# eora-ai/torchok

Measured on AMD Instinct MI355X. Metric: images/sec (node) ResNet-50 224px bs256/GPU; step p50 ms, higher is better.
Workload: dtype bf16

## Files before the change

include/tok.h:

```cpp
#ifndef TOK_H_
#define TOK_H_

#include <stddef.h>
#include <stdint.h>

#ifdef __cplusplus
extern "C" {
#endif

typedef enum tok_status {
  TOK_OK = 0,
  TOK_ERR_INVALID = -1,
  TOK_ERR_LAUNCH = -2,
  TOK_ERR_WORKSPACE = -3
} tok_status;

typedef enum tok_dtype { TOK_F32 = 0, TOK_F16 = 1, TOK_BF16 = 2 } tok_dtype;

typedef struct tok_conv_desc {
  int32_t n, h, w, c;
  int32_t k;
  int32_t r, s;
  int32_t p, q;
  int32_t stride, pad;
// ... 23 lines not shown
  int32_t k, r, s, c, k_pad, s_pad, c_pad;
  int32_t block_start;
} tok_pack_item;
int tok_pack_item_blocks(const tok_pack_item* item );
int tok_pack_weights_batched(const tok_pack_item* items_dev, int n_items, int total_blocks, void* stream);


int tok_conv_fwd_stat_rows(const tok_conv_desc* d);
int tok_conv_fwd(const tok_conv_desc* d, const void* x, const void* w, const float* bias,
                 void* y, float* stats, void* stream);
int tok_conv_dgrad(const tok_conv_desc* d, const void* dy, const void* w_dgrad, void* dx,
                   int accumulate, void* stream);
int tok_conv_dgrad_stat_rows(const tok_conv_desc* d);
int tok_conv_dgrad_bnstats(const tok_conv_desc* d, const void* dy, const void* w_dgrad, void* dx,
                           int accumulate, const void* bn_y, const uint8_t* bn_mask, float* partial,
                           void* stream);
int tok_bn_gram_finalize(const float* Z, const float* zsum, const float* w, int64_t count, int p, int k,
                         const float* gamma, const float* beta, float* running_mean, float* running_var,
                         int64_t* num_batches_tracked, float momentum, float eps, float* mean, float* rstd,
                         float* scale, float* shift, float* wz ,
                         void* stream);
int tok_conv_fwd_bn_apply(const tok_conv_desc* d, const void* x, const void* w, const float* scale, const float* shift,
                          const void* shortcut , int relu, void* out, uint8_t* mask ,
                          void* stream);
int tok_conv_dgrad_maskstore(const tok_conv_desc* d, const void* dy, const void* w_dgrad, void* dx, int accumulate,
                             const uint8_t* mask, float* partial, void* stream);
int tok_relu_mask_reduce(const void* dout, const uint8_t* mask, int64_t m, int c, void* dz, float* partial, void* stream);
int tok_bn3_bwd_prepare(const float* G, const float* w, const float* wz, const float* zsum, const float* partial, int rows,
                        int64_t count, int p, int k, const float* gamma, const float* mean, const float* rstd,
                        float* dgamma, float* dbeta, int param_accumulate, float* coef, float* dw, int dw_accumulate,
                        void* wa, void* wb, float* cvec, float* ws ,
                        void* stream);
size_t tok_bn3_bwd_prepare_ws_floats(int p, int k);
int tok_conv_dgrad_bias(const tok_conv_desc* d, const void* dy, const void* w_dgrad, const float* bias, void* dx,
                        int accumulate, const void* bn_y, const uint8_t* bn_mask, float* partial, void* stream);
int tok_subsample2_fwd(const void* x, int n, int h, int w, int c, void* out, void* stream);
int tok_subsample2_bwd(const void* dsub, int n, int h, int w, int c, void* dx, int accumulate, void* stream);
int tok_conv_dgrad_subacc_ok(const tok_conv_desc* d);
int tok_conv_dgrad_subacc(const tok_conv_desc* d, const void* dy, const void* w_dgrad, void* dx, const void* dsub,
                          const void* bn_y , const uint8_t* mask ,
                          float* partial , int mask_store, void* stream);
int tok_conv_dgrad2_ok(const tok_conv_desc* d1, const tok_conv_desc* d2);
int tok_conv_dgrad2(const tok_conv_desc* d1, const void* dy1, const void* w1_dgrad, const tok_conv_desc* d2, const void* dy2,
                    const void* w2_dgrad, const float* bias , void* dx, int accumulate,
                    const void* bn_y , const uint8_t* bn_mask , float* partial ,
                    void* stream);
size_t tok_conv_wgrad_ws_bytes(const tok_conv_desc* d);
int tok_conv_wgrad(const tok_conv_desc* d, const void* x, const void* dy, float* dw,
                   int k_real, int c_real, void* ws, size_t ws_bytes, int accumulate,
                   void* stream);
int tok_conv_wgrad_bias_ok(const tok_conv_desc* d);
size_t tok_conv_wgrad_bias_ws_bytes(const tok_conv_desc* d);
int tok_conv_wgrad_bias(const tok_conv_desc* d, const void* x, const void* dy, float* dw, int k_real, int c_real,
                        void* ws, size_t ws_bytes, int accumulate, float* dbias, int bias_accumulate, void* stream);


int tok_bn_finalize(const float* stats, int rows, int64_t count, int c, int c_real,
                    const float* gamma, const float* beta,
                    float* running_mean, float* running_var, int64_t* nbt,
                    float momentum, float eps,
                    float* mean, float* rstd, float* scale, float* shift, void* stream);
int tok_bn_eval_coeffs(const float* gamma, const float* beta, const float* running_mean,
                       const float* running_var, float eps, int c, int c_real,
                       float* scale, float* shift, void* stream);
int tok_bn_stats_rows(int64_t m, int c);
int tok_bn_stats(const void* y, int64_t m, int c, float* stats, void* stream);
// ... 313 lines not shown
```

torchok_amd/_C.py:

```python
import ctypes
import os
from ctypes import POINTER, Structure, c_char_p, c_float, c_int, c_int32, c_int64, c_size_t, c_void_p

_HERE = os.path.dirname(os.path.abspath(__file__))
LIB_PATH = os.environ.get('TOK_LIB') or os.path.join(_HERE, 'lib', 'libtok_gfx950.so')

TOK_F32, TOK_F16, TOK_BF16 = 0, 1, 2
TOK_CE_LOSS_FLOATS = 2050


class ConvDesc(Structure):
    _fields_ = [('n', c_int32), ('h', c_int32), ('w', c_int32), ('c', c_int32),
                ('k', c_int32), ('r', c_int32), ('s', c_int32),
                ('p', c_int32), ('q', c_int32),
                ('stride', c_int32), ('pad', c_int32), ('s_pad', c_int32)]


class PackItem(Structure):
    _fields_ = [('src', c_void_p), ('dst_fwd', c_void_p), ('dst_dgrad', c_void_p),
                ('k', c_int32), ('r', c_int32), ('s', c_int32), ('c', c_int32),
                ('k_pad', c_int32), ('s_pad', c_int32), ('c_pad', c_int32), ('block_start', c_int32)]


TOK_GRAD_CLIP_MAX_PARTIALS = 1024
# ... 27 lines not shown
    'tok_bn_eval_coeffs': (c_int, [_P, _P, _P, _P, c_float, c_int, c_int, _P, _P, _P]),
    'tok_bn_stats_rows': (c_int, [c_int64, c_int]),
    'tok_bn_stats': (c_int, [_P, c_int64, c_int, _P, _P]),
    'tok_bn_act_fwd': (c_int, [_P, _P, _P, _P, c_int, _P, _P, c_int64, c_int, _P]),
    'tok_bn_act_fwd_colsum_rows': (c_int, [c_int64, c_int]),
    'tok_event_create': (_P, []),
    'tok_event_destroy': (c_int, [_P]),
    'tok_next_launch_event': (c_int, [_P]),
    'tok_stream_wait_event': (c_int, [_P, _P]),
    'tok_bn_act_fwd_colsum': (c_int, [_P, _P, _P, _P, c_int, _P, _P, c_int64, c_int, _P, _P]),
    'tok_bn_bwd_rows': (c_int, [c_int64, c_int]),
    'tok_bn_bwd_reduce': (c_int, [_P, _P, _P, _P, _P, _P, _P, c_int, c_int64, c_int, _P, _P]),
    'tok_bn_bwd_finalize': (c_int, [_P, c_int, c_int64, c_int, c_int, _P, _P, _P, _P, _P, _P, c_int, c_int, _P]),
    'tok_bn_bwd_apply': (c_int, [_P, _P, _P, _P, _P, _P, c_int, _P, _P, c_int, c_int64, c_int, _P]),
    'tok_bn_hswish_fwd': (c_int, [_P, _P, _P, _P, c_int64, c_int, _P]),
    'tok_bn_hswish_bwd_reduce': (c_int, [_P, _P, _P, _P, _P, _P, c_int64, c_int, _P, _P]),
    'tok_bn_hswish_bwd_apply': (c_int, [_P, _P, _P, _P, _P, _P, c_int64, c_int, _P]),
    'tok_maxpool3x3s2_fwd': (c_int, [_P, _P, _P, c_int, c_int, c_int, c_int, _P]),
    'tok_maxpool3x3s2_bwd': (c_int, [_P, _P, _P, c_int, c_int, c_int, c_int, c_int, _P]),
    'tok_avgpool2x2_fwd': (c_int, [_P, _P, c_int, c_int, c_int, c_int, _P]),
    'tok_avgpool2x2_bwd': (c_int, [_P, _P, c_int, c_int, c_int, c_int, c_int, _P]),
    'tok_gap_fwd': (c_int, [_P, _P, c_int, c_int, c_int, _P]),
    'tok_gap_bwd': (c_int, [_P, _P, c_int, c_int, c_int, c_int, _P]),
    'tok_global_pool_fwd': (c_int, [_P, _P, _P, c_int, c_int, c_int, c_int, c_int, _P]),
    'tok_global_pool_bwd': (c_int, [_P, _P, _P, c_int, c_int, c_int, c_int, c_int, c_int, _P]),
    'tok_colsum': (c_int, [_P, c_int64, c_int, c_int, _P, c_int, _P]),
    'tok_bn_gram_finalize': (c_int, [_P, _P, _P, c_int64, c_int, c_int, _P, _P, _P, _P, _P, c_float, c_float, _P, _P, _P, _P, _P, _P]),
    'tok_conv_fwd_bn_apply': (c_int, [POINTER(ConvDesc), _P, _P, _P, _P, _P, c_int, _P, _P, _P]),
    'tok_conv_dgrad_maskstore': (c_int, [POINTER(ConvDesc), _P, _P, _P, c_int, _P, _P, _P]),
    'tok_relu_mask_reduce': (c_int, [_P, _P, c_int64, c_int, _P, _P, _P]),
    'tok_bn3_bwd_prepare': (c_int, [_P, _P, _P, _P, _P, c_int, c_int64, c_int, c_int, _P, _P, _P, _P, _P, c_int, _P, _P, c_int,
                                    _P, _P, _P, _P, _P]),
    'tok_bn3_bwd_prepare_ws_floats': (c_size_t, [c_int, c_int]),
    'tok_conv_dgrad_bias': (c_int, [POINTER(ConvDesc), _P, _P, _P, _P, c_int, _P, _P, _P, _P]),
    'tok_conv_dgrad2_ok': (c_int, [POINTER(ConvDesc), POINTER(ConvDesc)]),
    'tok_conv_dgrad2': (c_int, [POINTER(ConvDesc), _P, _P, POINTER(ConvDesc), _P, _P, _P, _P, c_int, _P, _P, _P, _P]),
    'tok_subsample2_fwd': (c_int, [_P, c_int, c_int, c_int, c_int, _P, _P]),
    'tok_subsample2_bwd': (c_int, [_P, c_int, c_int, c_int, c_int, _P, c_int, _P]),
    'tok_conv_dgrad_subacc_ok': (c_int, [POINTER(ConvDesc)]),
    'tok_conv_dgrad_subacc': (c_int, [POINTER(ConvDesc), _P, _P, _P, _P, _P, _P, _P, c_int, _P]),
    'tok_softmax_ce_fwd': (c_int, [_P, _P, c_int, c_int, c_int, c_int64, _P, _P, _P, _P]),
    'tok_softmax_ce_bwd': (c_int, [_P, _P, _P, _P, _P, c_int, c_int, c_int, c_int64, _P, _P]),
    'tok_softmax_ce_smooth_fwd': (c_int, [_P, _P, c_int, c_int, c_int, c_int64, c_float, _P, _P, _P, _P]),
    'tok_softmax_ce_smooth_bwd': (c_int, [_P, _P, _P, _P, _P, c_int, c_int, c_int, c_int64, c_float, _P, _P]),
    'tok_upsample_ce_serves': (c_int, [c_int, c_int]),
    'tok_upsample_ce_fwd': (c_int, [_P, c_int, c_int, c_int, c_int, c_int, c_int, c_int, _P, c_int64, _P, _P, _P, _P]),
    'tok_upsample_ce_bwd': (c_int, [_P, c_int, c_int, c_int, c_int, c_int, c_int, c_int, _P, c_int64, _P, _P, _P, _P, c_int, _P]),
    'tok_dice_rows': (c_int, [c_int64]),
    'tok_dice_fwd': (c_int, [_P, _P, c_int64, c_int, c_int, c_int, c_float, c_float, c_int, _P, c_int, _P, _P, _P, _P]),
    'tok_dice_bwd': (c_int, [_P, _P, _P, _P, c_int64, c_int, c_int, c_int, _P, _P]),
    'tok_bce_logits_fwd': (c_int, [_P, _P, c_int64, c_int, c_int, c_float, c_int, _P, _P]),
    'tok_bce_logits_bwd': (c_int, [_P, _P, _P, _P, c_int64, c_int, c_int, c_float, c_int, _P, _P]),
    'tok_relevance_matrix_multilabel': (c_int, [_P, _P, c_int, c_int, c_int, _P, _P]),
    'tok_embed_reg_fwd': (c_int, [_P, c_int, c_int, c_int, c_int, _P, _P, _P]),
    'tok_embed_reg_bwd': (c_int, [_P, _P, _P, c_float, c_int, c_int, c_int, c_int, _P, _P]),
    'tok_regression_loss_fwd': (c_int, [_P, _P, c_int64, c_int, c_float, c_int, _P, _P]),
    'tok_regression_loss_bwd': (c_int, [_P, _P, _P, c_int64, c_int, c_float, c_int, _P, _P]),
    'tok_confusion_update': (c_int, [_P, _P, _P, c_int64, c_int, c_int, c_int64, _P, _P]),
    'tok_cls_stats_update': (c_int, [_P, _P, _P, c_int64, c_int, c_int, c_int64, _P, _P]),
    'tok_l2norm_fwd': (c_int, [_P, _P, _P, c_int, c_int, c_int, c_int, c_float, _P]),
    'tok_l2norm_bwd': (c_int, [_P, _P, _P, _P, c_int, c_int, c_int, c_int, c_int, _P]),
    'tok_arcface_margin_fwd': (c_int, [_P, _P, c_int, c_int, c_int, c_float, c_float, c_float, c_float, c_int, c_float, _P, _P]),
    'tok_arcface_margin_bwd': (c_int, [_P, _P, _P, c_int, c_int, c_int, c_float, c_float, c_float, c_float, c_int, c_float, _P, _P]),
    'tok_relevance_matrix': (c_int, [_P, _P, c_int, c_int, _P, _P]),
    'tok_contrastive_fwd': (c_int, [_P, _P, _P, c_int, c_int, c_int, c_int, c_float, _P, _P, _P, _P]),
    'tok_contrastive_bwd': (c_int, [_P, _P, _P, _P, _P, c_int, c_int, c_int, c_int, c_float, _P, _P, c_int, _P]),
# ... 136 lines not shown
```

torchok_amd/csrc/conv_common.h:

```cpp
#pragma once
#include "tok_common.h"

struct FastDiv {
  uint32_t mul, shift;
};
static inline FastDiv make_fastdiv(uint32_t d) {
  FastDiv f;
  if (d <= 1) { f.mul = 0; f.shift = 0; return f; }
  uint32_t l = 0;
  while ((1ull << l) < d) ++l;
  f.mul = (uint32_t)((((1ull << 32) * ((1ull << l) - d)) / d) + 1);
  f.shift = l;
  return f;
}
__device__ __forceinline__ uint32_t fdiv(uint32_t n, FastDiv f) {
  return (uint32_t)(((uint64_t)__umulhi(n, f.mul) + n) >> f.shift);
}

struct ConvArgs {
  const bf16* x;
  const bf16* w;
  bf16* y;
  const float* bias;
  float* stats;
// ... 17 lines not shown
  int stride, pad;
  int M, PQ, Ktot, KT;
  int gridM, gridN;
  int accumulate, uniform_taps;
  uint32_t x_bytes, w_bytes;
  uint32_t s_bytes;
  FastDiv fd_pq, fd_q;
  unsigned long long* timing;
  int stat_rows;
  int cls_M[4], cls_nw[4], cls_hw[4];
  FastDiv cls_fd_hw[4], cls_fd_w[4];
};


bool conv_win_serves(const ConvArgs& a);
int conv_win_grid(int gridM, int gridN);
void conv_win_tiles(const ConvArgs& a, int* gridM, int* gridN);
int conv_win_launch(ConvArgs& a, hipStream_t st);
bool conv_s2d_serves(const ConvArgs& a, int stride, int pad);
int conv_s2d_grid(int gridM, int gridN);
void conv_s2d_tiles(const ConvArgs& a, int* gridM, int* gridN);
int conv_s2d_launch(ConvArgs& a, hipStream_t st);

bool gemm256_geometry(const ConvArgs& a);
bool gemm256_modes(const ConvArgs& a);
bool gemm256_serves(const ConvArgs& a);
int gemm256_rows(const ConvArgs& a);
int gemm256_launch(ConvArgs& a, hipStream_t st);

bool stem_win_serves(const ConvArgs& a);
int stem_win_launch(ConvArgs& a, int stat_rows, hipStream_t st);
bool stem_wgrad_serves(const tok_conv_desc* d);
int stem_wgrad_launch(const tok_conv_desc* d, const void* x, const void* dy, float* ws, int slabs, hipStream_t st);
```

torchok_amd/csrc/conv_wgrad.hip:

```cpp
#include "tok_common.h"
#include "conv_common.h"
#include <type_traits>
#include <stdlib.h>

namespace {

struct WgradArgs {
  const bf16* x;
  const bf16* dy;
  float* ws;
  int H, W, C, K, R, S, P, Q, stride, pad;
  int M, PQ, HW, Ktot;
  int tilesN, tilesK, splitM, mchunk;
  uint32_t x_bytes, dy_bytes;
  uint32_t pq_mul, pq_shift, q_mul, q_shift;
  float* cs;
  int cs_cols;
  int adv_q, adv_p;
  size_t cs_stride, ws_stride;
};

__device__ __forceinline__ uint32_t magic_div(uint32_t n, uint32_t mul, uint32_t shift) {
  return (uint32_t)(((uint64_t)__umulhi(n, mul) + n) >> shift);
}
// ... 1131 lines not shown
    return true;
  }();
  (void)attr_set;
  hipLaunchKernelGGL((conv_wgrad_ring_kernel<TN, TK>), dim3(a.tilesN * a.tilesK * a.splitM), dim3(256), smem, st, a);
}

template <int TN, int TK, bool C4, int MS, bool PWK>
void launch_wgrad_pw(const WgradArgs& a, hipStream_t st) {
  constexpr int smem = 2 * MS * ((TN + 16) * 2 + (TK + 16) * 2);
  static const bool attr_set = [&] {
    (void)hipFuncSetAttribute(reinterpret_cast<const void*>(&conv_wgrad_kernel<TN, TK, C4, MS, PWK>),
                              hipFuncAttributeMaxDynamicSharedMemorySize, smem);
    return true;
  }();
  (void)attr_set;
  hipLaunchKernelGGL((conv_wgrad_kernel<TN, TK, C4, MS, PWK>), dim3(a.tilesN * a.tilesK * a.splitM), dim3(256),
                     smem, st, a);
}

template <int TN, int TK, bool C4, int MS>
void launch_wgrad_ms(const WgradArgs& a, hipStream_t st) {
  if constexpr (!C4) {
    if (a.R == 1 && a.S == 1 && a.stride == 1 && a.pad == 0) { launch_wgrad_pw<TN, TK, C4, MS, true>(a, st); return; }
  }
  launch_wgrad_pw<TN, TK, C4, MS, false>(a, st);
}

template <int TN, int TK, bool C4>
void launch_wgrad(const WgradArgs& a, hipStream_t st, int ms) {
  if (ms == 64) launch_wgrad_ms<TN, TK, C4, 64>(a, st);
  else launch_wgrad_ms<TN, TK, C4, 32>(a, st);
}

}

extern "C" size_t tok_conv_wgrad_ws_bytes(const tok_conv_desc* d) {
  if (d == nullptr) return 0;
  const Plan p = make_plan(d);
  return (size_t)p.splitM * d->k * d->r * d->s_pad * d->c * sizeof(float);
}

extern "C" int tok_conv_wgrad_bias_ok(const tok_conv_desc* d) {
  if (d == nullptr || d->c == 4) return 0;
  return make_plan(d).ring ? 1 : 0;
}

extern "C" size_t tok_conv_wgrad_bias_ws_bytes(const tok_conv_desc* d) {
  if (d == nullptr) return 0;
  const Plan p = make_plan(d);
  return tok_conv_wgrad_ws_bytes(d) + (size_t)p.splitM * d->k * sizeof(float);
}

namespace {
int wgrad_impl(const tok_conv_desc* d, const void* x, const void* dy, float* dw, int k_real, int c_real, void* ws, size_t ws_bytes,
               int accumulate, float* dbias, int bias_accumulate, void* stream);
}

extern "C" int tok_conv_wgrad(const tok_conv_desc* d, const void* x, const void* dy, float* dw,
                              int k_real, int c_real, void* ws, size_t ws_bytes, int accumulate,
                              void* stream) {
  return wgrad_impl(d, x, dy, dw, k_real, c_real, ws, ws_bytes, accumulate, nullptr, 0, stream);
}

extern "C" int tok_conv_wgrad_bias(const tok_conv_desc* d, const void* x, const void* dy, float* dw, int k_real, int c_real,
                                   void* ws, size_t ws_bytes, int accumulate, float* dbias, int bias_accumulate, void* stream) {
  TOK_CHECK_ARG(dbias != nullptr, "tok_conv_wgrad_bias: dbias must not be null");
// ... 122 lines not shown
```

torchok_amd/csrc/unit3.hip:

```cpp
#include "tok_common.h"

namespace {

__device__ __forceinline__ float round_bf16(float v) { return bf2f(f2bf(v)); }

template <bool TRANS_A, bool ROUND_A, bool ROUND_B>
__global__ __launch_bounds__(256) void gemm_f32_kernel(const float* __restrict__ A, int lda, const float* __restrict__ B, int ldb,
                                                       int M, int N, int L, float* __restrict__ C, int ldc, int epi, int split,
                                                       bf16* __restrict__ Cb, int ldcb, float* __restrict__ cvec) {
  __shared__ float As[16][64 + 4];
  __shared__ float Bs[16][64 + 4];
  const int tid = threadIdx.x;
  const int i0 = blockIdx.y * 64, j0 = blockIdx.x * 64;
  const int ti = tid >> 4, tj = tid & 15;
  const int lchunk = ((L + (int)gridDim.z - 1) / (int)gridDim.z + 15) / 16 * 16;
  const int lbeg = blockIdx.z * lchunk;
  const int lend = min(L, lbeg + lchunk);
  if (gridDim.z > 1) C += (size_t)blockIdx.z * M * ldc;
  float acc[4][4];
#pragma unroll
  for (int r = 0; r < 4; ++r)
#pragma unroll
    for (int c = 0; c < 4; ++c) acc[r][c] = 0.f;
  for (int l0 = lbeg; l0 < lend; l0 += 16) {
#pragma unroll
    for (int e = 0; e < 4; ++e) {
      const int idx = tid + e * 256;
      int ii, ll;
      if (TRANS_A) { ii = idx & 63; ll = idx >> 6; }
      else { ll = idx & 15; ii = idx >> 4; }
      const int gi = i0 + ii, gl = l0 + ll;
      float v = 0.f;
      if (gi < M && gl < lend) v = TRANS_A ? A[(size_t)gl * lda + gi] : A[(size_t)gi * lda + gl];
// ... 278 lines not shown
    const float m1 = (float)(a1 * inv_m), m2 = (float)(sx * inv_m);
    const float g = gamma[k], rs = rstd[k], mu = mean[k];
    const float c1 = g * rs;
    const float c2 = -c1 * rs * m2;
    const float c3 = -c1 * m1 - c2 * mu;
    if (lane == 0) {
      const float sdz = (float)a1, sdzx = (float)sx;
      if (dgamma != nullptr) dgamma[k] = param_accumulate ? dgamma[k] + sdzx : sdzx;
      if (dbeta != nullptr) dbeta[k] = param_accumulate ? dbeta[k] + sdz : sdz;
      coef[k] = c1; coef[K + k] = c2; coef[2 * K + k] = c3;
      At[(size_t)k * (P + 1) + P] = c3;
    }
    for (int p = lane; p < P; p += 64) {
      const size_t o = (size_t)k * P + p;
      const float wq = round_bf16(w[o]);
      const float v = fmaf(c1, G[o], fmaf(c2, T[o], c3 * zsum[p]));
      dw[o] = dw_accumulate ? dw[o] + v : v;
      At[(size_t)k * (P + 1) + p] = c2 * wq;
      wl[c * P + p] = c1 * wq;
    }
  }
  __syncthreads();
  for (int i = tid; i < P * (PR_CH / 8); i += 1024) {
    const int p = i / (PR_CH / 8), h = i % (PR_CH / 8);
    if (k0 + h * 8 + 8 <= K) {
      bf16x8 o;
#pragma unroll
      for (int e = 0; e < 8; ++e) o[e] = f2bf(wl[(h * 8 + e) * P + p]);
      stg16(wa + (size_t)p * K + k0 + h * 8, o);
    }
  }
}

inline int mr_geo(int c, int& cge, int& rpb) {
  const int cg_total = c / 8;
  cge = cg_total < 256 ? cg_total : 256;
  rpb = 256 / cge;
  return cg_total;
}

}

extern "C" int tok_bn_bwd_rows(int64_t m, int c);

namespace {
inline int gemm_splits(int M, int N, int L) {
  const int tiles = tok_cdiv(N, 64) * tok_cdiv(M, 64);
  int s = tok_cdiv(512, tiles);
  const int maxs = L / 64 > 0 ? L / 64 : 1;
  if (s > maxs) s = maxs;
  return s < 1 ? 1 : s;
}

template <bool TA, bool RA, bool RB>
void launch_gemm(const float* A, int lda, const float* B, int ldb, int M, int N, int L, float* C, int ldc, int epi, int split,
                 bf16* Cb, int ldcb, float* cvec, float* parts, hipStream_t st) {
  const int splits = parts != nullptr ? gemm_splits(M, N, L) : 1;
  if (splits == 1) {
    hipLaunchKernelGGL((gemm_f32_kernel<TA, RA, RB>), dim3(tok_cdiv(N, 64), tok_cdiv(M, 64), 1), dim3(256), 0, st, A, lda, B,
                       ldb, M, N, L, C, ldc, epi, split, Cb, ldcb, cvec);
    return;
  }
  hipLaunchKernelGGL((gemm_f32_kernel<TA, RA, RB>), dim3(tok_cdiv(N, 64), tok_cdiv(M, 64), splits), dim3(256), 0, st, A, lda, B,
                     ldb, M, N, L, parts, N, 0, 0, nullptr, 0, nullptr);
  const size_t total = (size_t)M * N;
  hipLaunchKernelGGL(gemm_splits_reduce_kernel, dim3((int)((total + 255) / 256 < 1024 ? (total + 255) / 256 : 1024)), dim3(256),
                     0, st, parts, splits, M, N, C, ldc, epi, split, Cb, ldcb, cvec);
}
}

extern "C" int tok_bn_gram_finalize(const float* Z, const float* zsum, const float* w, int64_t count, int p, int k,
                                    const float* gamma, const float* beta, float* running_mean, float* running_var,
                                    int64_t* num_batches_tracked, float momentum, float eps, float* mean, float* rstd,
                                    float* scale, float* shift, float* wz, void* stream) {
  TOK_CHECK_ARG(Z && zsum && w && gamma && beta && mean && rstd && scale && shift && wz, "tok_bn_gram_finalize: null pointer");
  TOK_CHECK_ARG(count > 0 && p > 0 && k > 0, "tok_bn_gram_finalize: bad sizes");
  TOK_CHECK_ARG((running_mean == nullptr) == (running_var == nullptr), "tok_bn_gram_finalize: running stats go together");
  if (tok_dbg_skip(4)) return TOK_OK;
  hipStream_t st = tok_stream(stream);
  if (p == 64 || p == 128 || p == 256) {
    hipLaunchKernelGGL(bn_gram_finalize_block_kernel, dim3(k), dim3(256), 0, st, wz, Z, zsum, w, count, p, k, gamma, beta,
                       running_mean, running_var, num_batches_tracked, momentum, eps, mean, rstd, scale, shift);
    TOK_CHECK_LAUNCH("tok_bn_gram_finalize");
    return TOK_OK;
  }
  launch_gemm<false, true, false>(w, p, Z, p, k, p, p, wz, p, 0, 0, nullptr, 0, nullptr, nullptr, st);
  TOK_CHECK_LAUNCH("tok_bn_gram_finalize(gemm)");
  hipLaunchKernelGGL(bn_gram_finalize_kernel, dim3(tok_cdiv(k, 4)), dim3(256), 0, st, wz, zsum, w, count, p, k, gamma, beta,
                     running_mean, running_var, num_batches_tracked, momentum, eps, mean, rstd, scale, shift);
  TOK_CHECK_LAUNCH("tok_bn_gram_finalize");
  return TOK_OK;
}

extern "C" int tok_relu_mask_reduce(const void* dout, const uint8_t* mask, int64_t m, int c, void* dz, float* partial,
                                    void* stream) {
  TOK_CHECK_ARG(dout && dz && partial && m > 0 && c > 0 && c % 8 == 0, "tok_relu_mask_reduce: bad args");
  int cge, rpb;
  mr_geo(c, cge, rpb);
  const int rows = tok_bn_bwd_rows(m, c);
  hipLaunchKernelGGL(relu_mask_reduce_kernel, dim3(rows), dim3(256), 0, tok_stream(stream), (const bf16*)dout, mask, m, c, cge,
                     rpb, (bf16*)dz, partial);
  TOK_CHECK_LAUNCH("tok_relu_mask_reduce");
  return TOK_OK;
}

extern "C" size_t tok_bn3_bwd_prepare_ws_floats(int p, int k) {
  return (size_t)k * (p + 1) + (size_t)gemm_splits(p + 1, p, k) * (p + 1) * p;
}

extern "C" int tok_bn3_bwd_prepare(const float* G, const float* w, const float* wz, const float* zsum, const float* partial,
                                   int rows, int64_t count, int p, int k, const float* gamma, const float* mean,
                                   const float* rstd, float* dgamma, float* dbeta, int param_accumulate, float* coef,
                                   float* dw, int dw_accumulate, void* wa, void* wb, float* cvec, float* ws, void* stream) {
  TOK_CHECK_ARG(G && w && wz && zsum && partial && gamma && mean && rstd && coef && dw && wa && wb && cvec && ws,
                "tok_bn3_bwd_prepare: null pointer");
  TOK_CHECK_ARG(rows > 0 && count > 0 && p > 0 && p <= 2048 && k > 0 && k % 8 == 0, "tok_bn3_bwd_prepare: bad sizes");
  if (tok_dbg_skip(4)) return TOK_OK;
  hipStream_t st = tok_stream(stream);
  const size_t smem = (size_t)PR_CH * p * sizeof(float);
  static const bool attr_set = [&] {
    (void)hipFuncSetAttribute(reinterpret_cast<const void*>(&bn3_prepare_rows_kernel), hipFuncAttributeMaxDynamicSharedMemorySize,
                              PR_CH * 2048 * 4);
    return true;
// ... 17 lines not shown
```

torchok_amd/engine/functional.py:

```python
import weakref
from typing import Optional

import os

import torch
from torch import nn

from .. import _C
from .core import _ms as _core_ms
from . import paramgrad as PG
from .core import BF16, Node, Region, TTensor, await_ready, donate_grad, grad_target, is_last_contribution, pad8, ptr, stream_ptr

F32 = torch.float32



class _Packs:
    __slots__ = ('fwd', 'dgrad', 'bias', 'key', 'synced', 'dims')

    def __init__(self):
        self.fwd = None
        self.dgrad = None
        self.bias = None
        self.key = None
# ... 326 lines not shown
                                                       ptr(partial), 1, st), 'tok_conv_dgrad_subacc')
                    prod.masked_partial = (partial, rows)
                elif fuse:
                    partial = torch.empty((2, rows, x.cp), dtype=F32, device=g.device)
                    _C.check(lib.tok_conv_dgrad_subacc(d, ptr(dy), ptr(self.pk.dgrad), ptr(tgt), ptr(sub), ptr(prod.y),
                                                       ptr(prod.mask) if prod.relu else None, ptr(partial), 0, st),
                             'tok_conv_dgrad_subacc')
                    prod.fused_partial = (partial, rows)
                else:
                    _C.check(lib.tok_conv_dgrad_subacc(d, ptr(dy), ptr(self.pk.dgrad), ptr(tgt), ptr(sub), None, None, None, 0,
                                                       st), 'tok_conv_dgrad_subacc')
            elif mask_fuse:
                rows = lib.tok_conv_dgrad_stat_rows(d)
                partial = torch.empty((2, rows, x.cp), dtype=F32, device=g.device)
                _C.check(lib.tok_conv_dgrad_maskstore(d, ptr(dy), ptr(self.pk.dgrad), ptr(tgt), acc, ptr(prod.mask),
                                                      ptr(partial), st), 'tok_conv_dgrad_maskstore')
                prod.masked_partial = (partial, rows)
            elif fuse:
                rows = lib.tok_conv_dgrad_stat_rows(d)
                partial = torch.empty((2, rows, x.cp), dtype=F32, device=g.device)
                _C.check(lib.tok_conv_dgrad_bnstats(d, ptr(dy), ptr(self.pk.dgrad), ptr(tgt), acc, ptr(prod.y),
                                                    ptr(prod.mask) if prod.relu else None, ptr(partial), st),
                         'tok_conv_dgrad_bnstats')
                prod.fused_partial = (partial, rows)
            else:
                _C.check(lib.tok_conv_dgrad(d, ptr(dy), ptr(self.pk.dgrad), ptr(tgt), acc, st), 'tok_conv_dgrad')



FUSE_UNIT3 = os.environ.get('TOK_FUSE_UNIT3', '1') != '0'
UNIT3_MIN_ROWS = int(os.environ.get('TOK_UNIT3_MIN_ROWS', '100000'))


def _pointwise_desc(x: TTensor, k: int) -> _C.ConvDesc:
    n, h, w, cp = x.shape
    return _C.ConvDesc(n, h, w, cp, k, 1, 1, h, w, 1, 0, 1)


def _colsum_f32(t: torch.Tensor, m: int, c: int) -> torch.Tensor:
    out = torch.empty(c, dtype=F32, device=t.device)
    PG.colsum(t, m, c, out, 0, two_pass=m > 4096, n_real=c)
    return out


class _Unit3Node(Node):
    needs_backward = True

    def __init__(self):
        self.x = self.out = self.shortcut = self.mask = None
        self.relu = True
        self.masked_partial = None

    def release(self):
        self.x = self.out = self.shortcut = self.mask = self.masked_partial = None
        self.mean = self.rstd = self.wz = self.zsum = self.pk = None

    def backward(self):
        lib, st = _C.lib(), stream_ptr()
        out: TTensor = self.out
        g = out.grad
        if g is None:
            return
        conv, bn, d, x, sc = self.conv, self.bn, self.desc, self.x, self.shortcut
        kp, p = d.k, d.c
        m = d.n * d.p * d.q
        dev = g.device
# ... 49 lines not shown
                part2 = torch.empty((2, rows2, p), dtype=F32, device=dev)
            _C.check(lib.tok_conv_dgrad2(d, ptr(dz), ptr(wa), dpp, ptr(x.data), ptr(wb), ptr(cvec), ptr(tgt), acc,
                                         ptr(prod.y) if fuse else None, ptr(prod.mask) if (fuse and prod.relu) else None,
                                         ptr(part2), st), 'tok_conv_dgrad2')
            if fuse:
                prod.fused_partial = (part2, rows2)
            if self.region is not None:
                self.region.keep_until_join(dz, wa, wb, cvec, G, scratch)
            return
        _C.check(lib.tok_conv_dgrad(d, ptr(dz), ptr(wa), ptr(tgt), acc, st), 'tok_conv_dgrad')
        if fuse:
            rows2 = lib.tok_conv_dgrad_stat_rows(dpp)
            part2 = torch.empty((2, rows2, p), dtype=F32, device=dev)
            _C.check(lib.tok_conv_dgrad_bias(dpp, ptr(x.data), ptr(wb), ptr(cvec), ptr(tgt), 1, ptr(prod.y),
                                             ptr(prod.mask) if prod.relu else None, ptr(part2), st), 'tok_conv_dgrad_bias')
            prod.fused_partial = (part2, rows2)
        else:
            _C.check(lib.tok_conv_dgrad_bias(dpp, ptr(x.data), ptr(wb), ptr(cvec), ptr(tgt), 1, None, None, None, st),
                     'tok_conv_dgrad_bias')
        if self.region is not None:
            self.region.keep_until_join(dz, wa, wb, cvec, G, scratch)


def _unit3_forward(region: Region, x: TTensor, conv: nn.Conv2d, bn: nn.BatchNorm2d, shortcut: Optional[TTensor], kp: int,
                   relu: bool) -> TTensor:
    lib, st = _C.lib(), stream_ptr()
    dev = x.data.device
    if bn.momentum is None:
        raise NotImplementedError('BatchNorm momentum=None (cumulative average)')
    d = _pointwise_desc(x, kp)
    p = x.cp
    m = d.n * d.p * d.q
    pk = get_packs(conv.weight, None, kp, 1, p, want_dgrad=False, refresh=True)
    dz_ = _pointwise_desc(x, p)
    zz = PG.weight_grad(dz_, x.data, x.data, p, p)[0]
    if x.colsum_part is not None:
        part, nrows = x.colsum_part
        zsum = torch.empty(p, dtype=F32, device=x.data.device)
        _C.check(lib.tok_colsum_f32(ptr(part), nrows, p, ptr(zsum), 0, st), 'tok_colsum_f32')
        x.colsum_part = None
    else:
        zsum = _colsum_f32(x.data, m, p)
    mean, rstd, scale, shift = (torch.empty(kp, dtype=F32, device=dev) for _ in range(4))
    wz = torch.empty((kp, p), dtype=F32, device=dev)
    track = bn.training and bn.track_running_stats and bn.running_mean is not None
    _C.check(lib.tok_bn_gram_finalize(ptr(zz), ptr(zsum), ptr(conv.weight), m, p, kp, ptr(bn.weight), ptr(bn.bias),
                                      ptr(bn.running_mean) if track else None, ptr(bn.running_var) if track else None,
                                      ptr(bn.num_batches_tracked) if track else None, float(bn.momentum), float(bn.eps),
                                      ptr(mean), ptr(rstd), ptr(scale), ptr(shift), ptr(wz), st), 'tok_bn_gram_finalize')
    out_data = torch.empty((d.n, d.p, d.q, kp), dtype=BF16, device=dev)
    training = region.grad_mode and (conv.weight.requires_grad or x.requires_grad or bn.weight.requires_grad
                                     or (shortcut is not None and shortcut.requires_grad))
    mask = torch.empty((m, kp // 8), dtype=torch.uint8, device=dev) if (training and relu) else None
    _C.check(lib.tok_conv_fwd_bn_apply(d, ptr(x.data), ptr(pk.fwd), ptr(scale), ptr(shift),
                                       ptr(shortcut.data) if shortcut is not None else None, int(relu), ptr(out_data),
                                       ptr(mask), st), 'tok_conv_fwd_bn_apply')
    out = TTensor(out_data, kp, requires_grad=bool(training))
    if training:
        node = _Unit3Node()
        node.x, node.out, node.shortcut, node.mask, node.relu = x, out, shortcut, mask, relu
        node.conv, node.bn, node.desc, node.pk = conv, bn, d, pk
        node.mean, node.rstd, node.wz, node.zsum = mean, rstd, wz, zsum
        out.node = node
        if x.requires_grad:
            x.uses += 1
        if shortcut is not None and shortcut.requires_grad:
            shortcut.uses += 1
        region.add(node)
    return out


FUSE_STEM_POOL = os.environ.get('TOK_FUSE_STEM_POOL', '1') != '0'
STEM_POOLED_STATS = os.environ.get('TOK_STEM_POOLED_STATS', '1') != '0'


# ... 524 lines not shown
```

Measured before the change: 14410.

## Add dedicated symmetric Gram kernel with fused column sums for unit3 BN stats

Replaces the generic wgrad(x, x) call used to form the Gram matrix X^T X in the fused conv+BN forward with a dedicated MFMA kernel for p=64/128. The kernel uses a 3-stage LDS ring fed by buffer_load_lds and transposed LDS reads, exploits symmetry so diagonal waves read only once and one wave mirrors tiles, and computes column sums alongside via MFMA against a ones vector. This removes the separate colsum pass and part of the redundant Gram work. The cost is new specialized code with split-M workspace and a fold kernel, and it only applies when m is at least 100000.

```diff
diff --git a/include/tok.h b/include/tok.h
--- a/include/tok.h
+++ b/include/tok.h
@@ -79,6 +79,8 @@
                         void* wa, void* wb, float* cvec, float* ws ,
                         void* stream);
 size_t tok_bn3_bwd_prepare_ws_floats(int p, int k);
+size_t tok_gram_ws_bytes(int64_t m, int p);
+int tok_gram(const void* x, int64_t m, int p, float* z, float* zsum , float* ws, void* stream);
 int tok_conv_dgrad_bias(const tok_conv_desc* d, const void* dy, const void* w_dgrad, const float* bias, void* dx,
                         int accumulate, const void* bn_y, const uint8_t* bn_mask, float* partial, void* stream);
 int tok_subsample2_fwd(const void* x, int n, int h, int w, int c, void* out, void* stream);
diff --git a/torchok_amd/_C.py b/torchok_amd/_C.py
--- a/torchok_amd/_C.py
+++ b/torchok_amd/_C.py
@@ -83,6 +83,8 @@
     'tok_bn3_bwd_prepare': (c_int, [_P, _P, _P, _P, _P, c_int, c_int64, c_int, c_int, _P, _P, _P, _P, _P, c_int, _P, _P, c_int,
                                     _P, _P, _P, _P, _P]),
     'tok_bn3_bwd_prepare_ws_floats': (c_size_t, [c_int, c_int]),
+    'tok_gram_ws_bytes': (c_size_t, [c_int64, c_int]),
+    'tok_gram': (c_int, [_P, c_int64, c_int, _P, _P, _P, _P]),
     'tok_conv_dgrad_bias': (c_int, [POINTER(ConvDesc), _P, _P, _P, _P, c_int, _P, _P, _P, _P]),
     'tok_conv_dgrad2_ok': (c_int, [POINTER(ConvDesc), POINTER(ConvDesc)]),
     'tok_conv_dgrad2': (c_int, [POINTER(ConvDesc), _P, _P, POINTER(ConvDesc), _P, _P, _P, _P, c_int, _P, _P, _P, _P]),
diff --git a/torchok_amd/csrc/conv_common.h b/torchok_amd/csrc/conv_common.h
--- a/torchok_amd/csrc/conv_common.h
+++ b/torchok_amd/csrc/conv_common.h
@@ -73,3 +73,7 @@
 int stem_win_launch(ConvArgs& a, int stat_rows, hipStream_t st);
 bool stem_wgrad_serves(const tok_conv_desc* d);
 int stem_wgrad_launch(const tok_conv_desc* d, const void* x, const void* dy, float* ws, int slabs, hipStream_t st);
+
+void wgrad_pointwise_split(int64_t m, int p, int* splitM, int* mchunk);
+void wgrad_fold_flat_launch(const float* ws, float* dw, int splitM, size_t slab, size_t stride, float* extra, int extra_n,
+                            int extra_pad, hipStream_t st);
diff --git a/torchok_amd/csrc/conv_wgrad.hip b/torchok_amd/csrc/conv_wgrad.hip
--- a/torchok_amd/csrc/conv_wgrad.hip
+++ b/torchok_amd/csrc/conv_wgrad.hip
@@ -1187,6 +1187,21 @@
   else launch_wgrad_ms<TN, TK, C4, 32>(a, st);
 }
 
+}
+
+void wgrad_pointwise_split(int64_t m, int p, int* splitM, int* mchunk) {
+  tok_conv_desc d;
+  d.n = 1; d.h = 1; d.w = (int)m; d.c = p; d.k = p; d.r = 1; d.s = 1; d.p = 1; d.q = (int)m; d.stride = 1; d.pad = 0; d.s_pad = 1;
+  const Plan pl = make_plan(&d);
+  *splitM = pl.splitM;
+  *mchunk = pl.mchunk;
+}
+
+void wgrad_fold_flat_launch(const float* ws, float* dw, int splitM, size_t slab, size_t stride, float* extra, int extra_n,
+                            int extra_pad, hipStream_t st) {
+  const size_t nb = (slab / 4 + 15) / 16;
+  hipLaunchKernelGGL(wgrad_reduce_flat_kernel, dim3((int)(nb < 4096 ? nb : 4096)), dim3(256), 0, st, ws, dw, splitM, slab, 0, stride,
+                     extra, extra_n, extra_pad, 0);
 }
 
 extern "C" size_t tok_conv_wgrad_ws_bytes(const tok_conv_desc* d) {
diff --git a/torchok_amd/csrc/unit3.hip b/torchok_amd/csrc/unit3.hip
--- a/torchok_amd/csrc/unit3.hip
+++ b/torchok_amd/csrc/unit3.hip
@@ -1,4 +1,5 @@
 #include "tok_common.h"
+#include "conv_common.h"
 
 namespace {
 
@@ -343,6 +344,178 @@
   }
 }
 
+struct GramArgs {
+  const bf16* x;
+  float* ws;
+  float* cs;
+  int M, splitM, mchunk;
+  uint32_t x_bytes;
+  size_t stride;
+};
+
+__device__ __forceinline__ u32x2 gram_tr_read(uint32_t lds_addr) {
+  u32x2 v;
+  asm volatile("ds_read_b64_tr_b16 %0, %1" : "=v"(v) : "v"(lds_addr));
+  return v;
+}
+
+template <int P>
+__global__ __launch_bounds__(256, 3) void gram_ring_kernel(GramArgs a) {
+  constexpr int MS = 32, NST = 3;
+  constexpr int CN = P / 8;
+  constexpr int RPP = 256 / CN;
+  constexpr int LOADS = MS / RPP;
+  constexpr int RS = P * 2;
+  constexpr int STAGE = MS * RS;
+  constexpr int SW = (CN / 2 - 1) < (RPP - 1) ? (CN / 2 - 1) : (RPP - 1);
+  constexpr int NT = P / 32;
+  static_assert(P == 64 || P == 128, "gram_ring_kernel: P is 64 or 128");
+
+  __shared__ __attribute__((aligned(16))) char smem[NST * STAGE];
+
+  const int tid = threadIdx.x;
+  const int lane = tid & 63;
+  const int wv = tid >> 6;
+  const int wn2 = wv & 1, wk2 = wv >> 1;
+  const int wave_u = __builtin_amdgcn_readfirstlane(wv);
+
+  const int split = tok_xcd_remap(blockIdx.x, a.splitM);
+  const int mstart = split * a.mchunk;
+  const int mend = min(a.M, mstart + a.mchunk);
+  const int steps = (mend - mstart + MS - 1) / MS;
+
+  const int col = tid % CN, row = tid / CN;
+  const int clog = col ^ ((row & SW) << 1);
+  int xm = mstart + row;
+
+  const __amdgpu_buffer_rsrc_t srd = __builtin_amdgcn_make_buffer_rsrc((void*)a.x, 0, a.x_bytes, 0x00020000);
+  typedef __attribute__((address_space(3))) void lds_void;
+
+  auto issue = [&](int dbuf) {
+    char* dst = smem + dbuf * STAGE + wave_u * 1024;
+#pragma unroll
+    for (int i = 0; i < LOADS; ++i) {
+      const int m = xm + i * RPP;
+      uint32_t off = m < mend ? ((uint32_t)m * (uint32_t)P + (uint32_t)(clog * 8)) * 2u : 0xFFFFFFF0u;
+      asm volatile("" : "+v"(off));
+      __builtin_amdgcn_raw_ptr_buffer_load_lds(srd, (lds_void*)(dst + i * RPP * RS), 16, off, 0, 0, 0);
+    }
+    xm += MS;
+  };
+
+  const int g = lane >> 4, li = lane & 15;
+  const int rrow = 4 * g + (li >> 2);
+  const int swz = ((rrow & SW) << 1) << 4;
+  auto colb = [&](int half, int i) { return ((half * (P / 2) + i * 16 + (li & 3) * 4) * 2) ^ swz; };
+
+  const bool mm = P == 64 || wv != 1;
+  const bool do_cs = a.cs != nullptr && (P == 64 ? wk2 == 0 : wv == 1);
+  f32x4 acc[NT][NT];
+#pragma unroll
+  for (int i = 0; i < NT; ++i)
+#pragma unroll
+    for (int j = 0; j < NT; ++j) acc[i][j] = (f32x4){0.f, 0.f, 0.f, 0.f};
+  f32x4 csa[NT];
+#pragma unroll
+  for (int i = 0; i < NT; ++i) csa[i] = (f32x4){0.f, 0.f, 0.f, 0.f};
+  const bf16 one_b = (bf16)1.0f;
+  const bf16x8 ones = {one_b, one_b, one_b, one_b, one_b, one_b, one_b, one_b};
+
+  typedef __attribute__((address_space(3))) char lds_char;
+  const uint32_t lds_base = (uint32_t)(size_t)(lds_char*)smem;
+  issue(0);
+  issue(1);
+  int cur = 0, nxt = 2;
+  for (int st = 0; st < steps; ++st) {
+    asm volatile("s_waitcnt vmcnt(%0) lgkmcnt(0)" ::"n"(LOADS) : "memory");
+    __builtin_amdgcn_s_barrier();
+    issue(nxt);
+    if (mm || do_cs) {
+      const uint32_t Xb = lds_base + cur * STAGE;
+      u32x2 ya[NT][2], xb[NT][2];
+#pragma unroll
+      for (int i = 0; i < NT; ++i) {
+        ya[i][0] = gram_tr_read(Xb + rrow * RS + colb(wn2, i));
+        ya[i][1] = gram_tr_read(Xb + (rrow + 16) * RS + colb(wn2, i));
+      }
+      const bool diag = wn2 == wk2;
+      if (!diag) {
+#pragma unroll
+        for (int j = 0; j < NT; ++j) {
+          xb[j][0] = gram_tr_read(Xb + rrow * RS + colb(wk2, j));
+          xb[j][1] = gram_tr_read(Xb + (rrow + 16) * RS + colb(wk2, j));
+        }
+      }
+      asm volatile("s_waitcnt lgkmcnt(0)" ::: "memory");
+      __builtin_amdgcn_sched_barrier(0);
+      bf16x8 af[NT];
+#pragma unroll
+      for (int i = 0; i < NT; ++i) af[i] = __builtin_bit_cast(bf16x8, (u32x4){ya[i][0][0], ya[i][0][1], ya[i][1][0], ya[i][1][1]});
+      if (diag) {
+#pragma unroll
+        for (int i = 0; i < NT; ++i)
+#pragma unroll
+          for (int j = 0; j < NT; ++j)
+            acc[i][j] = __builtin_amdgcn_mfma_f32_16x16x32_bf16(af[i], af[j], acc[i][j], 0, 0, 0);
+        if (P == 64 && do_cs) {
+#pragma unroll
+          for (int i = 0; i < NT; ++i) csa[i] = __builtin_amdgcn_mfma_f32_16x16x32_bf16(af[i], ones, csa[i], 0, 0, 0);
+        }
+      } else {
+        bf16x8 bfr[NT];
+#pragma unroll
+        for (int j = 0; j < NT; ++j) bfr[j] = __builtin_bit_cast(bf16x8, (u32x4){xb[j][0][0], xb[j][0][1], xb[j][1][0], xb[j][1][1]});
+        if (mm) {
+#pragma unroll
+          for (int i = 0; i < NT; ++i)
+#pragma unroll
+            for (int j = 0; j < NT; ++j)
+              acc[i][j] = __builtin_amdgcn_mfma_f32_16x16x32_bf16(af[i], bfr[j], acc[i][j], 0, 0, 0);
+          if (P == 64 && do_cs) {
+#pragma unroll
+            for (int i = 0; i < NT; ++i) csa[i] = __builtin_amdgcn_mfma_f32_16x16x32_bf16(af[i], ones, csa[i], 0, 0, 0);
+          }
+        } else {
+#pragma unroll
+          for (int i = 0; i < NT; ++i) {
+            acc[i][0] = __builtin_amdgcn_mfma_f32_16x16x32_bf16(af[i], ones, acc[i][0], 0, 0, 0);
+            acc[i][1] = __builtin_amdgcn_mfma_f32_16x16x32_bf16(bfr[i], ones, acc[i][1], 0, 0, 0);
+          }
+        }
+      }
+    }
+    cur = cur == NST - 1 ? 0 : cur + 1;
+    nxt = nxt == NST - 1 ? 0 : nxt + 1;
+  }
+  asm volatile("s_waitcnt vmcnt(0)" ::: "memory");
+
+  if (do_cs && li == 0) {
+    float* cs = a.cs + (size_t)split * a.stride;
+#pragma unroll
+    for (int i = 0; i < NT; ++i)
+#pragma unroll
+      for (int r = 0; r < 4; ++r) {
+        cs[wn2 * (P / 2) + i * 16 + g * 4 + r] = P == 64 ? csa[i][r] : acc[i][0][r];
+        if (P == 128) cs[wk2 * (P / 2) + i * 16 + g * 4 + r] = acc[i][1][r];
+      }
+  }
+  if (!mm) return;
+
+  float* out = a.ws + (size_t)split * a.stride;
+#pragma unroll
+  for (int i = 0; i < NT; ++i) {
+#pragma unroll
+    for (int j = 0; j < NT; ++j) {
+      const int kcol = wk2 * (P / 2) + j * 16 + li;
+      const int n0 = wn2 * (P / 2) + i * 16 + g * 4;
+#pragma unroll
+      for (int r = 0; r < 4; ++r) out[(size_t)(n0 + r) * P + kcol] = acc[i][j][r];
+      if (P == 128 && wv == 2)
+        *reinterpret_cast<f32x4*>(out + (size_t)kcol * P + n0) = acc[i][j];
+    }
+  }
+}
+
 inline int mr_geo(int c, int& cge, int& rpb) {
   const int cg_total = c / 8;
   cge = cg_total < 256 ? cg_total : 256;
@@ -400,6 +573,44 @@
   hipLaunchKernelGGL(bn_gram_finalize_kernel, dim3(tok_cdiv(k, 4)), dim3(256), 0, st, wz, zsum, w, count, p, k, gamma, beta,
                      running_mean, running_var, num_batches_tracked, momentum, eps, mean, rstd, scale, shift);
   TOK_CHECK_LAUNCH("tok_bn_gram_finalize");
+  return TOK_OK;
+}
+
+namespace {
+constexpr int GRAM_MIN_ROWS = 8 * 32;
+inline bool gram_geometry_ok(int64_t m, int p) {
+  return (p == 64 || p == 128) && m >= GRAM_MIN_ROWS && (unsigned long long)m * p * 2 < 0xFFFFFFF0ull;
+}
+}
+
+extern "C" size_t tok_gram_ws_bytes(int64_t m, int p) {
+  if (!gram_geometry_ok(m, p)) return 0;
+  int splitM, mchunk;
+  wgrad_pointwise_split(m, p, &splitM, &mchunk);
+  return (size_t)splitM * ((size_t)p * p + p) * sizeof(float);
+}
+
+extern "C" int tok_gram(const void* x, int64_t m, int p, float* z, float* zsum, float* ws, void* stream) {
+  TOK_CHECK_ARG(x && z && ws, "tok_gram: null pointer");
+  TOK_CHECK_ARG(p == 64 || p == 128, "tok_gram: p = %d is not served (64 or 128; other widths: tok_conv_wgrad on (x, x))", p);
+  TOK_CHECK_ARG(m >= GRAM_MIN_ROWS, "tok_gram: m = %lld below the plan's minimum of %d rows", (long long)m, GRAM_MIN_ROWS);
+  TOK_CHECK_ARG(gram_geometry_ok(m, p), "tok_gram: tensors of 4 GiB or more are not supported");
+  TOK_CHECK_ARG((((uintptr_t)z | (uintptr_t)ws) & 15) == 0, "tok_gram: z and ws must be 16-byte aligned");
+  if (tok_dbg_skip(16)) return TOK_OK;
+  hipStream_t st = tok_stream(stream);
+  GramArgs a;
+  a.x = (const bf16*)x; a.ws = ws; a.M = (int)m;
+  wgrad_pointwise_split(m, p, &a.splitM, &a.mchunk);
+  a.x_bytes = (uint32_t)((unsigned long long)m * p * 2);
+  const size_t slab = (size_t)p * p;
+  a.stride = zsum != nullptr ? slab + p : slab;
+  a.cs = zsum != nullptr ? ws + slab : nullptr;
+  if (p == 64) hipLaunchKernelGGL(gram_ring_kernel<64>, dim3(a.splitM), dim3(256), 0, st, a);
+  else hipLaunchKernelGGL(gram_ring_kernel<128>, dim3(a.splitM), dim3(256), 0, st, a);
+  TOK_CHECK_LAUNCH("tok_gram");
+  if (tok_dbg_skip(2)) return TOK_OK;
+  wgrad_fold_flat_launch(ws, z, a.splitM, slab, a.stride, zsum, p, p, st);
+  TOK_CHECK_LAUNCH("tok_gram(fold)");
   return TOK_OK;
 }
 
diff --git a/torchok_amd/engine/functional.py b/torchok_amd/engine/functional.py
--- a/torchok_amd/engine/functional.py
+++ b/torchok_amd/engine/functional.py
@@ -382,6 +382,9 @@
 UNIT3_MIN_ROWS = int(os.environ.get('TOK_UNIT3_MIN_ROWS', '100000'))
 
 
+GRAM_MIN_ROWS = 100000
+
+
 def _pointwise_desc(x: TTensor, k: int) -> _C.ConvDesc:
     n, h, w, cp = x.shape
     return _C.ConvDesc(n, h, w, cp, k, 1, 1, h, w, 1, 0, 1)
@@ -497,15 +500,23 @@
     p = x.cp
     m = d.n * d.p * d.q
     pk = get_packs(conv.weight, None, kp, 1, p, want_dgrad=False, refresh=True)
-    dz_ = _pointwise_desc(x, p)
-    zz = PG.weight_grad(dz_, x.data, x.data, p, p)[0]
+    zsum = None
     if x.colsum_part is not None:
         part, nrows = x.colsum_part
-        zsum = torch.empty(p, dtype=F32, device=x.data.device)
+        zsum = torch.empty(p, dtype=F32, device=dev)
         _C.check(lib.tok_colsum_f32(ptr(part), nrows, p, ptr(zsum), 0, st), 'tok_colsum_f32')
         x.colsum_part = None
+    if p in (64, 128) and m >= GRAM_MIN_ROWS:
+        zz = torch.empty((p, p), dtype=F32, device=dev)
+        ws = torch.empty(lib.tok_gram_ws_bytes(m, p) // 4, dtype=F32, device=dev)
+        cs = None
+        if zsum is None:
+            cs = zsum = torch.empty(p, dtype=F32, device=dev)
+        _C.check(lib.tok_gram(ptr(x.data), m, p, ptr(zz), ptr(cs), ptr(ws), st), 'tok_gram')
     else:
-        zsum = _colsum_f32(x.data, m, p)
+        zz = PG.weight_grad(_pointwise_desc(x, p), x.data, x.data, p, p)[0]
+        if zsum is None:
+            zsum = _colsum_f32(x.data, m, p)
     mean, rstd, scale, shift = (torch.empty(kp, dtype=F32, device=dev) for _ in range(4))
     wz = torch.empty((kp, p), dtype=F32, device=dev)
     track = bn.training and bn.track_running_stats and bn.running_mean is not None
```

Result: no change. 14410 (-0.0%).
